# una-dinosauria/Rayuela.jl

Hardware: AMD Instinct MI355X
Metric: ADC queries/sec (linscan_pq, exact top-1000) (higher is better)
Workload: dtype f32; 1 GPU; SIFT1M-shape PQ m=8 h=256 encode + ADC linscan; n_base_total=1000000, n_base_per_gpu=1000000, nq=10000, k=1000, d=128, m=8, h=256, generator=splitmix64 (rayuela.jl_amd/synth.py; seeds base 1234, codebooks 99, rotation 7), parallelism=single GPU

## Files before the change

### include/rayuela_hip.h

```cpp
#ifndef RAYUELA_HIP_H_
#define RAYUELA_HIP_H_

#include <stddef.h>
#include <stdint.h>

#ifdef __cplusplus
extern "C" {
#endif

#define RQ_OK 0
#define RQ_EINVAL (-1)
#define RQ_EUNSUPPORTED (-2)
#define RQ_ENODEVICE (-3)

#define RQ_MAX_H16 32767
#define RQ_MAX_K 65536

const char *rq_version(void);
const char *rq_last_error(void);
int rq_device_count(void);
int rq_set_device(int device);

void linscan_aqd_query(float *dists, unsigned int *res, unsigned char *codes, float *centers,
                       float *queries, int N, unsigned int NQ, int B, int K, int dim1codes,
// ... 119 lines not shown
int rq_encode_opq_bytes_i16(int16_t *codes1, const uint8_t *X, const float *R, const float *C, int64_t n,
                            int d, int m, int h);
typedef struct rq_dataset rq_dataset;
rq_dataset *rq_dataset_upload(const float *X, int64_t n, int d);
rq_dataset *rq_dataset_upload_bytes(const uint8_t *X, int64_t n, int d);
int rq_dataset_encode(rq_dataset *ds, uint8_t *codes, int16_t *codes1, const float *R, const float *C, int m, int h);
void rq_dataset_free(rq_dataset *ds);
int rq_rotate_T(float *RX, const float *R, const float *X, int d, int64_t n);

int rq_dev_encode_pq(uint8_t *codes, const float *X, const float *C, int64_t n, int d, int m,
                     int h, void *stream);
int rq_dev_rotate_T(float *RX, const float *R, const float *X, int d, int64_t n, void *stream);
const char *rq_last_encode_kernel(void);
int rq_last_encode_stats(uint64_t *out2);
const char *rq_last_scan_kernel(void);
int rq_dev_encode_pq_filter_w(uint8_t *codes, float *W, const float *X, const float *C, int64_t n, int d, int m,
                              int h, void *stream);
int rq_dev_encode_opq(uint8_t *codes, const float *X, const float *R, const float *C, int64_t n,
                      int d, int m, int h, void *stream);
int rq_dev_encode_pq_bytes(uint8_t *codes, const uint8_t *X, const float *C, int64_t n, int d, int m,
                           int h, void *stream);
int rq_dev_encode_opq_bytes(uint8_t *codes, const uint8_t *X, const float *R, const float *C, int64_t n,
                            int d, int m, int h, void *stream);
int rq_dev_rotate_T_bytes(float *RX, const float *R, const uint8_t *X, int d, int64_t n, void *stream);
int rq_dev_encode_pq_wide(int16_t *codes, const float *X, const float *C, int64_t n, int d, int m, int h, void *stream);
int rq_dev_encode_opq_wide(int16_t *codes, const float *X, const float *R, const float *C, int64_t n, int d, int m, int h,
                           void *stream);
int rq_dev_encode_rvq_wide(int16_t *codes, float *Xr, const float *codebooks, int64_t n, int d, int m, int h,
                           uint32_t *counts, void *stream);
int rq_dev_adc_lut(float *lut, const float *centers, const float *queries, int64_t nq, int m,
// ... 67 lines not shown
```

### rayuela.jl_amd/_lib.py

```python
import ctypes as C

import numpy as np
import os

_HERE = os.path.dirname(os.path.abspath(__file__))


class RayuelaHipError(RuntimeError):
    pass


def lib_path():
    return os.environ.get("RAYUELA_HIP_LIB", os.path.join(_HERE, "librayuela_hip.so"))


_vp, _i32, _i64, _u32, _u64 = C.c_void_p, C.c_int, C.c_int64, C.c_uint32, C.c_uint64

SIGNATURES = {
    "rq_version": (C.c_char_p, []),
    "rq_last_scan_kernel": (C.c_char_p, []),
    "rq_last_error": (C.c_char_p, []),
    "rq_device_count": (_i32, []),
    "rq_set_device": (_i32, [_i32]),
    "linscan_aqd_query": (None, [_vp, _vp, _vp, _vp, _vp, _i32, C.c_uint, _i32, _i32, _i32, _i32, _i32]),
    "linscan_aqd_query_extra_byte": (None, [_vp, _vp, _vp, _vp, _vp, _vp, _i32, _i32, _i32, _i32, _i32, _i32]),
    "linscan_aqd_cq_query_extra_byte": (None, [_vp, _vp, _vp, _vp, _vp, _i32, _i32, _i32, _i32, _i32, _i32]),
    "rq_linscan_lsq": (_i32, [_vp, _vp, _vp, _vp, _vp, _vp, _vp, _i64, _i64, _i32, _i32, _i32, _i32, _i32]),
    "rq_linscan_cq": (_i32, [_vp, _vp, _vp, _vp, _vp, _i64, _i64, _i32, _i32, _i32, _i32, _i32]),
    "rq_lsq_prepare": (_vp, [_vp, _vp, _vp, _i64, _i32, _i32, _i32]),
    "rq_lsq_search": (_i32, [_vp, _vp, _vp, _vp, _vp, _i64, _i32, _i32]),
    "rq_lsq_release": (None, [_vp]),
    "rq_lsq_prepare_cbnorms": (_vp, [_vp, _vp, _vp, _i32, _i64, _i32, _i32, _i32]),
    "rq_aq_norms": (_i32, [_vp, _vp, _vp, _i64, _i32, _i32, _i32]),
    "rq_dev_aq_norms": (_i32, [_vp, _vp, _vp, _i64, _i32, _i32, _i32, _vp]),
    "rq_quantize_norms": (_i32, [_vp, _vp, _vp, _vp, _vp, _i64, _i32, _i32, _i32, _i32]),
# ... 217 lines not shown
```

### rayuela.jl_amd/csrc/rq_api.hip

```cpp
#include <stdarg.h>
#include <stdlib.h>
#include <string.h>

#include <chrono>
#include <mutex>
#include <string>
#include <thread>

#include <vector>
#include "rq_internal.h"

namespace rq {

static thread_local char g_err[512] = "";
static thread_local unsigned g_err_seq = 0;
static thread_local double g_t_total = 0, g_t_h2d = 0, g_t_kernel = 0, g_t_d2h = 0;

int fail(int code, const char *fmt, ...) {
  va_list ap;
  va_start(ap, fmt);
  vsnprintf(g_err, sizeof(g_err), fmt, ap);
  va_end(ap);
  ++g_err_seq;
  return code;
// ... 350 lines not shown
  RQ_TRY(order_cache_of(stream, &h, &og, &sg));
  if (sg != 0) {
    void *state = nullptr;
    RQ_TRY(workspace(WS_ORDER_STATE, order_cache_state_bytes(), &state, stream));
    RQ_HIP(hipMemsetAsync(state, 0, 8 * sizeof(uint32_t), stream));
  }
  h->key_id = 0;
  ++h->uncached;
  order_set_call_queries(nq);
  const int orc = order_base(ocodes, operm, ord, codes, n, mp, stream);
  order_set_call_queries(0);
  return orc;
}

static int order_kept(bool *kept, const uint8_t **ocodes, const uint32_t **operm, const uint8_t *codes, int64_t n, int m, int mp,
                      int64_t nq, size_t snap_off, hipStream_t stream) {
  *kept = true;
  OrderTiling ot;
  scan_order_tiling(mp, &ot);
  const int bits = order_cached_key_bits(n, mp, ot);
  if (bits <= 0) return RQ_OK;
  void *ord = nullptr, *state = nullptr, *tmp = nullptr;
  int rc = workspace(WS_ORDER, snap_off + (size_t)n * mp, &ord, stream);
  if (is_oom(rc)) { forgive_oom(); *kept = false; return RQ_OK; }
  RQ_TRY(rc);
  RQ_TRY(workspace(WS_ORDER_STATE, order_cache_state_bytes(), &state, stream));
  RQ_TRY(workspace(WS_ORDER_TMP, order_scratch_bytes(n, bits), &tmp, stream));
  OrderCacheHost *h = nullptr;
  uint64_t og = 0, sg = 0;
  RQ_TRY(order_cache_of(stream, &h, &og, &sg));
  if (h->state_gen != sg) {
    RQ_HIP(hipMemsetAsync(state, 0, order_cache_state_bytes(), stream));
    h->state_gen = sg; h->order_gen = og; h->key_id = 0;
  } else if (h->order_gen != og) {
    RQ_HIP(hipMemsetAsync(state, 0, 8 * sizeof(uint32_t), stream));
    h->order_gen = og; h->key_id = 0;
  }
  ++h->consulted;
  uint8_t *dst = (uint8_t *)ord;
  uint32_t *pm = reinterpret_cast<uint32_t *>(dst + (order_base_bytes(n, mp) - (size_t)n * 4));
  RQ_TRY(order_rows_cached(dst, pm, dst + snap_off, codes, n, m, mp, tmp, ot, nq, (uint32_t *)state, h, stream));
  *ocodes = dst;
  *operm = pm;
  return RQ_OK;
}

int order_cache_stats(unsigned long long *out8) {
  if (!out8) return fail(RQ_EINVAL, "rq_order_cache_stats: null output");
  int dev = 0;
  RQ_HIP(hipGetDevice(&dev));
  DeviceLock launch_lock;
  RQ_HIP(hipDeviceSynchronize());
  std::lock_guard<std::mutex> lk(g_mu);
  DevCtx &c = g_dev[dev];
  for (int i = 0; i < 8; ++i) out8[i] = 0;
  for (int i = 0; i < MAX_STREAM_WS; ++i) {
// ... 16 lines not shown
  const bool padded = base && (base->padded || base->perm);
  if (nq <= 0) return RQ_OK;
  if (n < 1 || n >= (1LL << 31)) return fail(RQ_EINVAL, "n=%lld must be in [1, 2^31)", (long long)n);
  if (lut_mode < LUT_PQ || lut_mode > LUT_CQ) return fail(RQ_EINVAL, "lut_mode=%d", lut_mode);
  if (m < 1 || d < 1 || (lut_mode == LUT_PQ && (d < m || d % m != 0)))
    return fail(RQ_EINVAL, "scan needs d %% m == 0 (src/Linscan.jl:23 Cint(d/m)); got d=%d m=%d", d, m);
  if (k < 1) return fail(RQ_EUNSUPPORTED, "k=%d outside [1, n]", k);
  if (k > n) return fail(RQ_EINVAL, "k=%d > n=%lld (undefined in the reference, deps/src/linscan_aqd.cpp:91)", k, (long long)n);
  if ((uint64_t)id_offset + (uint64_t)n > 0xFFFFFFFFull) return fail(RQ_EINVAL, "row ids overflow uint32");
  if (id_base != 0 && id_base != 1) return fail(RQ_EINVAL, "id_base must be 0 or 1");
  if (!keys && (!dists || !ids)) return fail(RQ_EINVAL, "need dists+ids or keys");
  if (((uintptr_t)codes & 15) != 0) return fail(RQ_EINVAL, "codes pointer must be 16-byte aligned");
  DeviceInfo di;
  RQ_TRY(device_info(&di));
  DeviceLock launch_lock;
  const int mp = scan_padded_m(m);
  if (mp < 0) return fail(RQ_EUNSUPPORTED, "the ADC scan kernels cover 1 <= m <= 64 sub-quantizers; got m=%d", m);
  if (mp != m && !padded) {
    void *padded = nullptr;
    RQ_TRY(workspace(WS_PAD, (size_t)n * mp, &padded, stream));
    RQ_TRY(pad_codes_launch((uint8_t *)padded, codes, n, m, mp, stream));
    codes = (const uint8_t *)padded;
  }
  if (k > RQ_MAX_K)
    return bulk_scan(dists, ids, keys, codes, centers, queries, n, nq, m, d, k, id_offset, id_base, stream, lut_mode, row_bias,
                     perm, di.num_cu);
  const size_t order_cap = (size_t)std::max(0, tuning("ORDER_MAX_SCRATCH_MB", 2048)) * 1048576ull;
  if (!perm && !row_bias && order_pays(n, nq, k) && order_base_bytes(n, mp) + (size_t)n * 4 <= order_cap) {
    const uint8_t *ocodes = codes;
    const uint32_t *operm = nullptr;
    const size_t snap_off = (order_base_bytes(n, mp) + 255) & ~(size_t)255, snap_bytes = (size_t)n * mp;
    bool kept = false;
    int orc = RQ_OK;
    if (snap_off + snap_bytes + (size_t)n * 4 <= order_cap) orc = order_kept(&kept, &ocodes, &operm, codes, n, m, mp, nq, snap_off, stream);
    if (orc == RQ_OK && !kept) orc = order_in_call(&ocodes, &operm, codes, n, mp, nq, stream);
    if (orc == RQ_OK) {
      codes = ocodes;
      perm = operm;
    } else if (is_oom(orc)) {
      forgive_oom();
    } else {
      return orc;
    }
  }
  ScanPlan pl;
  RQ_TRY(scan_plan(pl, n, nq, m, d, k, di.num_cu, tuning("SCAN_SLICES", 0)));
  void *cand = nullptr, *counter = nullptr;
  RQ_TRY(workspace(WS_CAND, pl.cand_bytes, &cand, stream));
  RQ_TRY(workspace(WS_COUNTER, WS_COUNTER_BYTES, &counter, stream));
  const int64_t q_tail = std::min<int64_t>(nq, (int64_t)pl.whole * pl.qg);
  const bool sliced = pl.nslices > 1 && q_tail < nq;
  const bool both = keys && (dists || ids);
  void *part = nullptr;
  if (sliced) RQ_TRY(workspace(WS_KEYS, (size_t)(nq - q_tail) * pl.nslices * k * sizeof(uint64_t), &part, stream));
  void *normb = norm_prepared;
  if (lut_mode == LUT_LSQ && row_bias && !normb)
    RQ_TRY(workspace(WS_NORMB, lsq_norm_bytes(n), &normb, stream));
  RQ_TRY(scan_launch(pl, both ? nullptr : dists, both ? nullptr : ids, keys, (uint64_t *)part, codes, centers, queries,
                     n, nq, m, d, k, id_offset, id_base, (uint32_t *)counter, (uint64_t *)cand, stream, lut_mode,
                     row_bias, (uint8_t *)normb, perm, norm_prepared != nullptr));
  if (sliced) {
    const size_t off = (size_t)q_tail * k;
    RQ_TRY(merge_launch(both || !dists ? nullptr : dists + off, both || !ids ? nullptr : ids + off,
                        keys ? keys + off : nullptr, (const uint64_t *)part, nq - q_tail, (int)pl.nslices, k, id_base,
                        stream));
  }
  if (both) return merge_launch(dists, ids, nullptr, keys, nq, 1, k, id_base, stream);
  return RQ_OK;
}

template <class ScanFn>
static int scan_and_fetch(float *dists, uint32_t *ids, float *dd, uint32_t *di, int64_t nq, int k, ScanFn scan) {
  const int64_t hc = std::max(256, tuning("HOST_CHUNK", 4096));
  const int64_t chunk = (nq >= 2 * hc && tuning("HOST_OVERLAP", 1)) ? hc : nq;
  const size_t row = (size_t)k * 4;
// ... 326 lines not shown
  g_t_kernel = std::max(0.0, g_t_total - h2d - tail);
  return RQ_OK;
}

}

using namespace rq;

extern "C" {

#ifndef RQ_BUILD_ID
#define RQ_BUILD_ID "unknown"
#endif
const char *rq_version(void) { return "rayuela-hip 0.1 (gfx950) build " RQ_BUILD_ID; }
const char *rq_last_scan_kernel(void) { return last_scan_kernel_name(); }
const char *rq_last_error(void) { return g_err; }

int rq_device_count(void) {
  int n = 0;
  if (hipGetDeviceCount(&n) != hipSuccess) { (void)hipGetLastError(); return 0; }
  return n;
}

int rq_set_device(int device) {
  RQ_HIP(hipSetDevice(device));
  return RQ_OK;
}

int rq_set_tuning(const char *key, int value) {
  if (!key || !*key) return fail(RQ_EINVAL, "rq_set_tuning: empty key");
// ... 774 lines not shown
```

### rayuela.jl_amd/csrc/rq_internal.h

```cpp
#pragma once
#include <hip/hip_runtime.h>
#include <stdint.h>
#include <stdio.h>

#include <math.h>

#include <algorithm>

#include "../../include/rayuela_hip.h"

namespace rq {

int fail(int code, const char *fmt, ...) __attribute__((format(printf, 2, 3)));
int fail_hip(hipError_t e, const char *what, const char *file, int line);
inline bool is_oom(int rc) { return rc == (int)hipErrorOutOfMemory; }
void forgive_oom();

#define RQ_HIP(expr)                                                       \
  do {                                                                     \
    hipError_t _e = (expr);                                                \
    if (_e != hipSuccess) return ::rq::fail_hip(_e, #expr, __FILE__, __LINE__); \
  } while (0)

#define RQ_TRY(expr)            \
// ... 44 lines not shown
void set_timing(double total_ms, double h2d_ms, double kernel_ms, double d2h_ms);

struct ScanPlan {
  int qg, blk;
  uint32_t ngroups, nslices, rows_per_slice, whole;
  uint32_t cap, trigger, p2, scratch_keys, grid, sample;
  size_t cand_bytes, gtab_off, bkt_off;
  bool lds_ok, bigk, spread;
  bool xcd;
};
int scan_plan(ScanPlan &pl, int64_t n, int64_t nq, int m, int d, int K, int num_cu, int force_slices);
int scan_launch(const ScanPlan &pl, float *dists, uint32_t *ids, uint64_t *keys, uint64_t *part, const uint8_t *codes,
                const float *centers, const float *queries, int64_t n, int64_t nq, int m, int d, int K,
                uint32_t id_offset, int id_base, uint32_t *work_counter, uint64_t *cand,
                hipStream_t stream, int lut_mode = 0, const float *row_bias = nullptr, uint8_t *norm_buf = nullptr,
                const uint32_t *perm = nullptr, bool norm_ready = false);
const char *last_scan_kernel_name();
void set_last_scan_kernel(const char *name);
size_t lsq_norm_bytes(int64_t n);
int lsq_norm_prepare(uint8_t *norm_buf, const uint8_t *codes, const float *centers, const float *row_bias, int64_t n,
                     int mp, int m_real, int d, hipStream_t stream);
enum { LUT_PQ = 0, LUT_LSQ = 1, LUT_CQ = 2 };
struct ScanBase {
  const uint32_t *perm = nullptr;
  uint8_t *norm_prepared = nullptr;
  bool padded = false;
};
int dev_linscan(float *dists, uint32_t *ids, uint64_t *keys, const uint8_t *codes, const float *centers,
                const float *queries, int64_t n, int64_t nq, int m, int d, int k, uint32_t id_offset,
                int id_base, hipStream_t stream, int lut_mode = LUT_PQ, const float *row_bias = nullptr,
                const ScanBase *base = nullptr);
bool order_pays(int64_t n, int64_t nq, int k);
// ... 10 lines not shown
int order_sample_stride();
uint32_t order_sample_rows(int64_t n, int blk, uint32_t *sgroups);
int gather_f32_launch(float *dst, const float *src, const uint32_t *perm, int64_t n, hipStream_t stream);
int order_rows_launch(uint8_t *dst, uint32_t *perm, const uint8_t *src, int64_t n, int mp, void *scratch,
                      const OrderTiling &t, hipStream_t stream);
struct OrderCacheHost {
  unsigned char key[768];
  uint32_t key_id = 0;
  uint32_t epoch = 0;
  uint64_t order_gen = 0, state_gen = 0;
  unsigned long long consulted = 0, uncached = 0;
};
size_t order_cache_state_bytes();
int order_cached_key_bits(int64_t n, int mp, const OrderTiling &t);
int order_rows_cached(uint8_t *dst, uint32_t *perm, uint8_t *snap, const uint8_t *src, int64_t n, int m, int mp, void *scratch,
                      const OrderTiling &t, int64_t nq, uint32_t *state, OrderCacheHost *h, hipStream_t stream);
int order_cache_stats(unsigned long long *out8);
int interleave_keys_launch(uint64_t *dst, const uint64_t *src, int64_t nq, int P, int k, size_t pstride, hipStream_t stream);
int scan_padded_m(int m);
int pad_codes_launch(uint8_t *dst, const uint8_t *src, int64_t n, int m, int mp, hipStream_t stream);
constexpr size_t BULK_SCRATCH_BYTES = (size_t)2 << 30;
constexpr size_t BULK_HOST_RESULT_BYTES = (size_t)256 << 20;
int bulk_scan(float *dists, uint32_t *ids, uint64_t *keys, const uint8_t *codes, const float *centers, const float *queries,
              int64_t n, int64_t nq, int m, int d, int k, uint32_t id_offset, int id_base, hipStream_t stream, int lut_mode,
              const float *row_bias, const uint32_t *perm, int num_cu);
int bulk_merge(float *dists, uint32_t *ids, uint64_t *keys_out, const uint64_t *keys_in, int64_t nq, int P, int K,
               int id_base, hipStream_t stream);
void bulk_plan(int64_t n, int64_t nq, int m, int k, int num_cu, int64_t *qg, int64_t *groups, int64_t *grid, int64_t *batch);
int merge_launch(float *dists, uint32_t *ids, uint64_t *keys_out, const uint64_t *keys_in, int64_t nq,
                 int P, int K, int id_base, hipStream_t stream);
int lut_launch(float *lut, const float *centers, const float *queries, int64_t nq, int m, int sub,
// ... 96 lines not shown
```

### rayuela.jl_amd/csrc/rq_order.hip

```cpp
#include "rq_internal.h"

#include <cmath>
#include <cstring>
#include <mutex>

namespace rq {

struct OrderParams {
  const uint8_t *src;
  uint8_t *dst;
  uint32_t *perm;
  uint32_t *rank;
  uint32_t *hist;
  uint32_t n;
  int mp;
  int ncoord;
  int nb[8];
  uint32_t nbins;
  uint32_t tile;
  uint32_t rpt;
  uint32_t group;
  uint32_t gran;
  uint32_t ngran;
  uint32_t weyl;
// ... 76 lines not shown
  if (lead) {
    g.state[OC_VERDICT] = v; g.state[OC_VEPOCH] = g.epoch;
    if (v == OCV_REBUILD) { g.state[OC_BUILT] = 0; g.state[OC_CNT + (g.balanced ? 2 : 1)] += 1; }
    else if (v == OCV_HIT) g.state[OC_CNT] += 1;
  }
  return v == OCV_REBUILD;
}
__device__ __forceinline__ bool order_gate_open(const OrderGate &g) {
  return !g.state || (g.state[OC_VEPOCH] == g.epoch && g.state[OC_VERDICT] == (g.role == 2 ? OCV_UPGRADE : OCV_REBUILD));
}
__device__ __forceinline__ bool order_gate_last(const OrderGate &g) {
  if (!order_gate_open(g)) return false;
  if (g.state && blockIdx.x == 0 && threadIdx.x == 0) { g.state[OC_BALANCED] = g.balanced; g.state[OC_BUILT] = g.key; }
  return true;
}
__device__ __forceinline__ void order_snapshot(const OrderGate &g, const uint8_t *src, size_t bytes) {
  if (!g.state || !g.snap || g.role != 1) return;
  const size_t nv = bytes / 16, nth = (size_t)gridDim.x * blockDim.x, t0 = (size_t)blockIdx.x * blockDim.x + threadIdx.x;
  for (size_t i = t0; i < nv; i += nth) reinterpret_cast<uint4 *>(g.snap)[i] = reinterpret_cast<const uint4 *>(src)[i];
  if (t0 == 0) for (size_t b = nv * 16; b < bytes; ++b) g.snap[b] = src[b];
}

__global__ __launch_bounds__(256) void order_check_kernel(const uint8_t *codes, const uint8_t *snap, size_t bytes, uint32_t *state,
                                                          uint32_t key, uint32_t epoch, uint32_t *zero, uint32_t nzero) {
  const size_t nth = (size_t)gridDim.x * blockDim.x, t0 = (size_t)blockIdx.x * blockDim.x + threadIdx.x;
  for (size_t i = t0; i < nzero; i += nth) zero[i] = 0u;
  if (state[OC_BUILT] != key) return;
  const size_t nv = bytes / 16;
  bool bad = false;
  for (size_t i = t0; i < nv; i += nth) {
    const uint4 a = reinterpret_cast<const uint4 *>(codes)[i], b = reinterpret_cast<const uint4 *>(snap)[i];
    bad |= ((a.x ^ b.x) | (a.y ^ b.y) | (a.z ^ b.z) | (a.w ^ b.w)) != 0u;
  }
  if (t0 == 0) for (size_t b = nv * 16; b < bytes; ++b) bad |= codes[b] != snap[b];
  if (bad) state[OC_MISS] = epoch;
}

__global__ __launch_bounds__(256) void order_zero_kernel(OrderParams p, uint32_t count, OrderGate g) {
  if (!order_gate_first(g)) return;
  order_snapshot(g, p.src, (size_t)p.n * p.mp);
  for (uint32_t i = blockIdx.x * blockDim.x + threadIdx.x; i < count; i += gridDim.x * blockDim.x) p.hist[i] = 0u;
// ... 92 lines not shown
      const uint32_t y = __shfl_up(x, off);
      if ((tid & 63u) >= (uint32_t)off) x += y;
    }
    if ((tid & 63u) == 63u) wsum[tid >> 6] = x;
  }
  __syncthreads();
  if (tid < ORDER_COARSE) {
    uint32_t base = 0;
    for (uint32_t w = 0; w < (tid >> 6); ++w) base += wsum[w];
    starts[tid] = base + x - v;
    if (tid == ORDER_COARSE - 1) starts[ORDER_COARSE] = base + x;
  }
  __syncthreads();
}

__global__ __launch_bounds__(ORDER_SMALL_THREADS) void order_coarse_count_kernel(OrderParams p, OrderSmall q, OrderGate g) {
  __shared__ uint32_t h[ORDER_COARSE];
  const uint32_t tid = threadIdx.x;
  if (!order_gate_first(g)) return;
  order_snapshot(g, p.src, (size_t)p.n * p.mp);
  if (tid < ORDER_COARSE) h[tid] = 0;
  __syncthreads();
  const uint32_t r0 = blockIdx.x * q.rows_per_wg, r1 = min(p.n, r0 + q.rows_per_wg);
  for (uint32_t i = r0 + tid; i < r1; i += ORDER_SMALL_THREADS)
    if (!order_in_prefix(p, i)) atomicAdd(&h[order_key_of(p, i) >> q.fine_bits], 1u);
  __syncthreads();
  if (tid < ORDER_COARSE && h[tid]) atomicAdd(&q.ctot[tid], h[tid]);
}

__global__ __launch_bounds__(ORDER_SMALL_THREADS) void order_coarse_scatter_kernel(OrderParams p, OrderSmall q, OrderGate g) {
  __shared__ uint32_t h[ORDER_COARSE], base[ORDER_COARSE], starts[ORDER_COARSE + 1];
  const uint32_t tid = threadIdx.x;
  if (!order_gate_open(g)) return;
  if (tid < ORDER_COARSE) h[tid] = 0;
  coarse_starts(starts, q.ctot);
  const uint32_t r0 = blockIdx.x * q.rows_per_wg, r1 = min(p.n, r0 + q.rows_per_wg);
  constexpr int PER = 4;
  uint32_t c[PER], lr[PER];
#pragma unroll
  for (int u = 0; u < PER; ++u) {
    const uint32_t i = r0 + u * ORDER_SMALL_THREADS + tid;
    c[u] = 0xffffffffu;
    if (i < r1) {
      if (order_in_prefix(p, i)) order_copy_row(p, i, order_sample_pos(p, i / p.stride));
      else { c[u] = order_key_of(p, i) >> q.fine_bits; lr[u] = atomicAdd(&h[c[u]], 1u); }
    }
  }
  __syncthreads();
  if (tid < ORDER_COARSE && h[tid]) base[tid] = starts[tid] + atomicAdd(&q.ctot[ORDER_COARSE + tid], h[tid]);
  __syncthreads();
#pragma unroll
  for (int u = 0; u < PER; ++u) {
    const uint32_t i = r0 + u * ORDER_SMALL_THREADS + tid;
    if (c[u] != 0xffffffffu) q.idx[base[c[u]] + lr[u]] = i;
  }
}

__global__ __launch_bounds__(ORDER_SMALL_THREADS) void order_fine_kernel(OrderParams p, OrderSmall q, OrderGate g) {
  __shared__ uint32_t f[ORDER_FINE_MAX], starts[ORDER_COARSE + 1], wsum[16];
  const uint32_t tid = threadIdx.x, nfine = 1u << q.fine_bits, fmask = nfine - 1u;
  if (!order_gate_last(g)) return;
  for (uint32_t i = tid; i < nfine; i += ORDER_SMALL_THREADS) f[i] = 0;
  coarse_starts(starts, q.ctot);
  const uint32_t b0 = starts[blockIdx.x], b1 = starts[blockIdx.x + 1];
  for (uint32_t i = b0 + tid; i < b1; i += ORDER_SMALL_THREADS) atomicAdd(&f[order_key_of(p, q.idx[i]) & fmask], 1u);
  __syncthreads();
  {
    const uint32_t v = tid < nfine ? f[tid] : 0u;
    uint32_t x = v;
#pragma unroll
// ... 90 lines not shown
#pragma unroll
        for (int i = 0; i < TPL; ++i)
          mine_st[i * 128 + (val[i] & 31u)] = (uint16_t)(((x[i] & 255u) + (fresh[i] ? 1u : 0u)) | (val[i] << 8));
        next += 1u;
      }
      myrank = lane == j ? newrank : myrank;
      __builtin_amdgcn_wave_barrier();
    }
    if (have) order_copy_row(p, row, order_deal(p, myrank));
    row = row_n;
#pragma unroll
    for (uint32_t i = 0; i < NW; ++i) w[i] = w_n[i];
  }
}

__global__ __launch_bounds__(ORDER_SMALL_THREADS) void order_fine_greedy_kernel(OrderParams p, OrderSmall q, OrderGate g) {
  __shared__ uint32_t f[ORDER_FINE_MAX], fst[ORDER_FINE_MAX + 1], starts[ORDER_COARSE + 1], wsum[16];
  extern __shared__ __attribute__((aligned(16))) uint32_t dyn[];
  const uint32_t tid = threadIdx.x, nfine = 1u << q.fine_bits, fmask = nfine - 1u;
  if (!order_gate_last(g)) return;
  for (uint32_t i = tid; i < nfine; i += ORDER_SMALL_THREADS) f[i] = 0;
  coarse_starts(starts, q.ctot);
  const uint32_t b0 = starts[blockIdx.x], b1 = starts[blockIdx.x + 1];
  const bool fits = b1 - b0 <= p.glist;
  for (uint32_t i = b0 + tid; i < b1; i += ORDER_SMALL_THREADS) atomicAdd(&f[order_key_of(p, q.idx[i]) & fmask], 1u);
  __syncthreads();
  {
    const uint32_t v = tid < nfine ? f[tid] : 0u;
    uint32_t x = v;
#pragma unroll
    for (int off = 1; off < 64; off <<= 1) {
      const uint32_t y = __shfl_up(x, off);
      if ((tid & 63u) >= (uint32_t)off) x += y;
    }
    if ((tid & 63u) == 63u) wsum[tid >> 6] = x;
    __syncthreads();
    uint32_t wb = 0;
    for (uint32_t w = 0; w < (tid >> 6); ++w) wb += wsum[w];
    if (tid < nfine) { f[tid] = b0 + wb + x - v; fst[tid] = b0 + wb + x - v; }
// ... 15 lines not shown
  }
  __syncthreads();
  const uint32_t wave = tid >> 6;
  if (wave >= p.gwaves) return;
  uint16_t *st = reinterpret_cast<uint16_t *>(reinterpret_cast<uint8_t *>(dyn + p.glist) + (size_t)wave * GREEDY_GROUPS * (uint32_t)p.gfree * 64u);
  const uint32_t window = GREEDY_GROUPS * p.group;
  for (uint32_t fb = wave; fb < nfine; fb += p.gwaves) {
    const uint32_t s0 = fst[fb], s1 = fst[fb + 1];
    for (uint32_t c0 = s0; c0 < s1;) {
      const uint32_t c1 = min(s1, c0 / p.group * p.group + window);
      if (p.mp == 8) greedy_chunk<8, 1>(p, list, b0, c0, c1, st);
      else greedy_chunk<16, 3>(p, list, b0, c0, c1, st);
      c0 = c1;
    }
  }
}

static uint32_t gcd_u32(uint32_t a, uint32_t b) { while (b) { const uint32_t t = a % b; a = b; b = t; } return a; }

int order_sample_stride() { return tuning("ORDER_SAMPLE_STRIDE", 16); }

uint32_t order_sample_rows(int64_t n, int blk, uint32_t *sgroups) {
  const int stride = order_sample_stride();
  uint32_t g = 0;
  if (stride >= 2 && blk > 0) g = (uint32_t)(n / ((int64_t)stride * blk));
  if (sgroups) *sgroups = g;
  return g * (uint32_t)blk;
}

static thread_local int64_t g_order_call_nq = 0;
// ... 114 lines not shown
    const OrderSmall &q = s.q;
    const uint32_t nwg = (uint32_t)((n + q.rows_per_wg - 1) / q.rows_per_wg);
    if (zero_counters) RQ_HIP(hipMemsetAsync(q.ctot, 0, 2 * ORDER_COARSE * 4, stream));
    hipLaunchKernelGGL(order_coarse_count_kernel, dim3(nwg), dim3(ORDER_SMALL_THREADS), 0, stream, p, q, g);
    RQ_HIP(hipGetLastError());
    hipLaunchKernelGGL(order_coarse_scatter_kernel, dim3(nwg), dim3(ORDER_SMALL_THREADS), 0, stream, p, q, g);
    RQ_HIP(hipGetLastError());
    if (s.greedy) {
      RQ_HIP(hipFuncSetAttribute(reinterpret_cast<const void *>(order_fine_greedy_kernel),
                                 hipFuncAttributeMaxDynamicSharedMemorySize, (int)s.lds));
      hipLaunchKernelGGL(order_fine_greedy_kernel, dim3(ORDER_COARSE), dim3(ORDER_SMALL_THREADS), s.lds, stream, p, q, g);
    } else {
      hipLaunchKernelGGL(order_fine_kernel, dim3(ORDER_COARSE), dim3(ORDER_SMALL_THREADS), 0, stream, p, q, g);
    }
    RQ_HIP(hipGetLastError());
    return RQ_OK;
  }
  const uint32_t ntiles = (p.nbins + ORDER_SCAN_TILE - 1) / ORDER_SCAN_TILE;
  const uint32_t grid = (uint32_t)std::min<int64_t>((n + 255) / 256, 256 * 16);
  if (g.state) {
    hipLaunchKernelGGL(order_zero_kernel, dim3(grid), dim3(256), 0, stream, p, p.nbins + ntiles, g);
    RQ_HIP(hipGetLastError());
  } else if (zero_counters) {
    RQ_HIP(hipMemsetAsync(p.hist, 0, (size_t)(p.nbins + ntiles) * 4, stream));
  }
  hipLaunchKernelGGL(order_rank_kernel, dim3(grid), dim3(256), 0, stream, p, g);
  RQ_HIP(hipGetLastError());
  hipLaunchKernelGGL(order_scan_tiles_kernel, dim3(ntiles), dim3(1024), 0, stream, p.hist, p.nbins, g);
  RQ_HIP(hipGetLastError());
  hipLaunchKernelGGL(order_scan_top_kernel, dim3(1), dim3(1024), 0, stream, p.hist + p.nbins, ntiles, g);
  RQ_HIP(hipGetLastError());
  hipLaunchKernelGGL(order_scatter_kernel, dim3(grid), dim3(256), 0, stream, p, g);
  RQ_HIP(hipGetLastError());
  return RQ_OK;
}

int order_rows_launch(uint8_t *dst, uint32_t *perm, const uint8_t *src, int64_t n, int mp, void *scratch,
                      const OrderTiling &t, hipStream_t stream) {
  OrderSet s;
  RQ_TRY(order_plan_set(s, n, mp, t));
  order_bind(s, dst, perm, src, scratch);
  OrderGate g;
  memset(&g, 0, sizeof(g));
  return order_run_set(s, g, true, stream);
}

struct OrderCacheKey {
  int64_t n;
// ... 1 lines not shown
  OrderSet plain, bal;
};
static_assert(sizeof(OrderCacheKey) <= sizeof(OrderCacheHost::key), "OrderCacheHost::key too small");

size_t order_cache_state_bytes() { return OC_WORDS * sizeof(uint32_t); }

int order_cached_key_bits(int64_t n, int mp, const OrderTiling &t) {
  int nb[8];
  order_set_call_queries(-1);
  const int bits = order_key_bits(n, mp, t, nb);
  order_set_call_queries(0);
  return bits;
}

int order_rows_cached(uint8_t *dst, uint32_t *perm, uint8_t *snap, const uint8_t *src, int64_t n, int m, int mp, void *scratch,
                      const OrderTiling &t, int64_t nq, uint32_t *state, OrderCacheHost *h, hipStream_t stream) {
  static uint32_t next_id = 0;
  static std::mutex id_mu;
  OrderCacheKey key;
  memset(&key, 0, sizeof(key));
  key.n = n; key.m = m; key.mp = mp;
  order_set_call_queries(-1);
  int rc = order_plan_set(key.plain, n, mp, t);
  order_set_call_queries(0);
  if (rc == RQ_OK) rc = order_plan_set(key.bal, n, mp, t);
  if (rc != RQ_OK) return rc;
  key.has_b = key.bal.greedy ? 1 : 0;
  if (!key.has_b) memset(&key.bal, 0, sizeof(key.bal));
  if (h->key_id == 0 || memcmp(h->key, &key, sizeof(key)) != 0) {
    std::lock_guard<std::mutex> lk(id_mu);
    if (++next_id == 0) ++next_id;
    h->key_id = next_id;
    memcpy(h->key, &key, sizeof(key));
  }
  if (++h->epoch == 0) ++h->epoch;
  const bool first_bal = key.has_b && !(nq > 0 && nq < tuning("ORDER_GREEDY_MIN_NQ", 16384));
  OrderSet first = first_bal ? key.bal : key.plain;
  order_bind(first, dst, perm, src, scratch);
  OrderGate g;
  memset(&g, 0, sizeof(g));
  g.state = state; g.snap = snap; g.key = h->key_id; g.epoch = h->epoch;
  g.role = 1; g.can_upgrade = key.has_b; g.balanced = first_bal;
  const size_t bytes = (size_t)n * mp;
  const uint32_t cgrid = (uint32_t)std::max<size_t>(1, std::min<size_t>((bytes / 16 + 511) / 512, 2048));
  const bool zero2 = first.two_level || g.can_upgrade;
  hipLaunchKernelGGL(order_check_kernel, dim3(cgrid), dim3(256), 0, stream, src, (const uint8_t *)snap, bytes, state, g.key, g.epoch,
                     reinterpret_cast<uint32_t *>(scratch) + n, zero2 ? 2u * ORDER_COARSE : 0u);
  RQ_HIP(hipGetLastError());
  RQ_TRY(order_run_set(first, g, false, stream));
  if (g.can_upgrade) {
    OrderSet up = key.bal;
    order_bind(up, dst, perm, src, scratch);
    g.role = 2; g.can_upgrade = 0; g.balanced = 1;
    RQ_TRY(order_run_set(up, g, false, stream));
  }
  return RQ_OK;
}

__global__ void gather_f32_kernel(float *__restrict__ dst, const float *__restrict__ src, const uint32_t *__restrict__ perm, uint32_t n) {
  for (uint32_t i = blockIdx.x * blockDim.x + threadIdx.x; i < n; i += gridDim.x * blockDim.x) dst[i] = src[perm[i]];
}

int gather_f32_launch(float *dst, const float *src, const uint32_t *perm, int64_t n, hipStream_t stream) {
  if (n <= 0) return RQ_OK;
  hipLaunchKernelGGL(gather_f32_kernel, dim3((uint32_t)std::min<int64_t>((n + 255) / 256, 4096)), dim3(256), 0, stream, dst, src, perm, (uint32_t)n);
  RQ_HIP(hipGetLastError());
  return RQ_OK;
}

}
```

### rayuela.jl_amd/csrc/rq_scan.hip

```cpp
#include "rq_internal.h"
#include "rq_topk.h"

#include "rq_scan_tables.h"
#include "rq_scan_filter.h"
#include "rq_scan_select.h"


namespace rq {

#define RQ_STAT_T() ((p.stats && threadIdx.x == 0) ? (unsigned long long)clock64() : 0ull)
#define RQ_STAT_ADD(slot, t0) do { if (p.stats && threadIdx.x == 0) atomicAdd(&p.stats[slot], (unsigned long long)clock64() - (t0)); } while (0)
#define RQ_STAT_INC(slot) do { if (p.stats && threadIdx.x == 0) atomicAdd(&p.stats[slot], 1ull); } while (0)

struct BucketFinishArgs {
  uint32_t cap, scratch_keys, nq, K, id_base;
  int bfin;
  float *dists;
  uint32_t *ids;
  unsigned long long *stats;
};
template <int M>
__device__ __noinline__ bool bucket_finish_item(ScanCtrl<ScanCfg<M>::QG> *ctrl_g, uint64_t *cand_wg, BucketFinishArgs p,
                                                uint64_t *scratch_g, int g, int gi, uint32_t q0, uint64_t *keys_base,
                                                uint32_t key_stride, uint32_t vseq_in, uint32_t *vseq_out) {
// ... 724 lines not shown
  const int lim = (int)((nbytes - i) < 8 ? (nbytes - i) : 8);
  for (int b = 0; b < lim; ++b) {
    uint64_t z = ((e0 + i + b) ^ seed) + 0x9E3779B97F4A7C15ull;
    z = (z ^ (z >> 30)) * 0xBF58476D1CE4E5B9ull;
    z = (z ^ (z >> 27)) * 0x94D049BB133111EBull;
    z = z ^ (z >> 31);
    out |= (z >> 56) << (8 * b);
  }
  if (lim == 8) *reinterpret_cast<uint64_t *>(codes + i) = out;
  else for (int b = 0; b < lim; ++b) codes[i + b] = (uint8_t)(out >> (8 * b));
}

static thread_local char g_last_scan_kernel[64] = "";
const char *last_scan_kernel_name() { return g_last_scan_kernel; }
void set_last_scan_kernel(const char *name) { snprintf(g_last_scan_kernel, sizeof(g_last_scan_kernel), "%s", name); }

template <int M>
static int launch_scan(ScanParams &p, const ScanPlan &plan, hipStream_t stream) {
  using Cfg = ScanCfg<M>;
  p.samp_end = 0; p.samp_stride = 16;
  if (p.perm) {
    uint32_t groups = 0;
    (void)order_sample_rows((int64_t)p.n, Cfg::BLK, &groups);
    p.samp_stride = (uint32_t)std::max(2, order_sample_stride());
    p.samp_end = groups * p.samp_stride * (uint32_t)Cfg::BLK;
  }
  constexpr int CTRL_BYTES = (sizeof(ScanCtrl<Cfg::QG>) + 15) & ~15;
  size_t lds = CTRL_BYTES + (size_t)std::max<size_t>(Cfg::LUT_LDS_BYTES + (size_t)Cfg::QG * p.d * 4 + Cfg::AUX_BYTES,
                                                     (size_t)p.scratch_keys * 8);
  if (p.bigk) lds = std::max<size_t>(lds, CTRL_BYTES + SS_LDS_BYTES);
// ... 191 lines not shown
  RQ_HIP(hipMemsetAsync(cn, 0, 16 * 256 * 4, stream));
  const uint32_t grid = (uint32_t)std::min<int64_t>(2048, (n + 255) / 256);
  hipLaunchKernelGGL(cnorm_kernel, dim3((m_real * 256 + 255) / 256), dim3(256), 0, stream, centers, m_real * 256, d, cn);
  hipLaunchKernelGGL(norm_residual_kernel, dim3(grid), dim3(256), 0, stream, row_bias, codes, (uint32_t)n, mp, m_real, cn, rho);
  hipLaunchKernelGGL(norm_minmax_kernel, dim3(grid), dim3(256), 0, stream, (const float *)rho, (uint32_t)n, info);
  hipLaunchKernelGGL(norm_info_kernel, dim3(1), dim3(1), 0, stream, info);
  hipLaunchKernelGGL(norm_quant_kernel, dim3(grid), dim3(256), 0, stream, (const float *)rho, (uint32_t)n, info, norm_buf);
  RQ_HIP(hipGetLastError());
  return RQ_OK;
}

int scan_launch(const ScanPlan &pl, float *dists, uint32_t *ids, uint64_t *keys, uint64_t *part, const uint8_t *codes,
                const float *centers, const float *queries, int64_t n, int64_t nq, int m, int d, int K,
                uint32_t id_offset, int id_base, uint32_t *work_counter, uint64_t *cand,
                hipStream_t stream, int lut_mode, const float *row_bias, uint8_t *norm_buf, const uint32_t *perm,
                bool norm_ready) {
  ScanParams p;
  p.perm = perm;
  p.samp_end = 0;
  p.codes = codes; p.centers = centers; p.queries = queries;
  p.n = (uint32_t)n; p.nq = (uint32_t)nq; p.sub = d / m; p.d = d; p.K = K;
  p.m_real = m;
  m = scan_padded_m(m);
  p.lut_mode = lut_mode; p.row_bias = row_bias;
  p.id_offset = id_offset; p.id_base = id_base;
  p.nslices = pl.nslices; p.rows_per_slice = pl.rows_per_slice; p.ngroups = pl.ngroups; p.whole = pl.whole;
  p.xcd_mode = pl.xcd ? 1u : 0u;
  {
    const uint32_t per_xcd = std::max(1u, pl.grid / 8u);
    const int rd = tuning("SCAN_XCD_ROUND", 0);
    p.xcd_round = rd > 0 ? (uint32_t)rd : pl.ngroups * ((per_xcd + pl.ngroups - 1u) / pl.ngroups);
// ... 22 lines not shown
  p.norm_bytes = nullptr; p.norm_info = nullptr; p.cnorm = nullptr;
  if (lut_mode == LUT_LSQ && row_bias && norm_buf && (m == 8 || m == 16) && tuning("SCAN_FILTER", 1) &&
      tuning("SCAN_FILTER_LSQ", 1)) {
    if (!norm_ready) RQ_TRY(lsq_norm_prepare(norm_buf, codes, centers, row_bias, n, m, p.m_real, d, stream));
    const size_t nb_bytes = ((size_t)n + 63) & ~(size_t)63;
    uint32_t *info = reinterpret_cast<uint32_t *>(norm_buf + nb_bytes);
    float *cn = reinterpret_cast<float *>(info + 8);
    p.norm_bytes = norm_buf;
    p.norm_info = reinterpret_cast<const float *>(info) + 4;
    p.cnorm = cn;
    p.filter = 1;
  }
  p.stats = tuning("SCAN_STATS", 0) ? reinterpret_cast<unsigned long long *>(work_counter + 16) : nullptr;
  p.dists = dists; p.ids = ids; p.keys = keys; p.part = part;
#if RQ_SCAN_PACE_BUILD
  if (p.pace) RQ_HIP(hipMemsetAsync(work_counter + 64, 0, WS_COUNTER_BYTES - 256, stream));
#endif
  RQ_HIP(hipMemsetAsync(work_counter, 0, p.stats ? 256 : 16 * sizeof(uint32_t), stream));
  switch (m) {
    case 2: return launch_scan<2>(p, pl, stream);
    case 4: return launch_scan<4>(p, pl, stream);
    case 8: return launch_scan<8>(p, pl, stream);
    case 16: return launch_scan<16>(p, pl, stream);
    case 32: return launch_scan<32>(p, pl, stream);
    case 64: return launch_scan<64>(p, pl, stream);
  }
  return fail(RQ_EUNSUPPORTED, "m=%d", m);
}

int merge_launch(float *dists, uint32_t *ids, uint64_t *keys_out, const uint64_t *keys_in, int64_t nq,
                 int P, int K, int id_base, hipStream_t stream) {
  if (P > 1 && K > RQ_MAX_K) return bulk_merge(dists, ids, keys_out, keys_in, nq, P, K, id_base, stream);
  MergeParams p;
// ... 79 lines not shown
```

Baseline: 5.503 million queries/s.

## Fuse order-cache first and upgrade passes and fold counter zeroing into check

The cached row-ordering path now runs the first and balanced-upgrade orderings as one set of three gated kernels that pick their parameter set from a device-side verdict, instead of launching both sets back to back. The scan work counter is zeroed inside the order check kernel, so the separate hipMemsetAsync before the scan is skipped when that happened. The aim is fewer kernel launches and memsets in front of the scan for each query batch, at the cost of more complex gate state handling. A launch counter API is added so the front launches can be inspected.

```diff
diff --git a/include/rayuela_hip.h b/include/rayuela_hip.h
--- a/include/rayuela_hip.h
+++ b/include/rayuela_hip.h
@@ -157,6 +157,7 @@
 const char *rq_last_encode_kernel(void);
 int rq_last_encode_stats(uint64_t *out2);
 const char *rq_last_scan_kernel(void);
+int rq_scan_front_launches(void);
 int rq_dev_encode_pq_filter_w(uint8_t *codes, float *W, const float *X, const float *C, int64_t n, int d, int m,
                               int h, void *stream);
 int rq_dev_encode_opq(uint8_t *codes, const float *X, const float *R, const float *C, int64_t n,
diff --git a/rayuela.jl_amd/_lib.py b/rayuela.jl_amd/_lib.py
--- a/rayuela.jl_amd/_lib.py
+++ b/rayuela.jl_amd/_lib.py
@@ -19,6 +19,7 @@
 SIGNATURES = {
     "rq_version": (C.c_char_p, []),
     "rq_last_scan_kernel": (C.c_char_p, []),
+    "rq_scan_front_launches": (_i32, []),
     "rq_last_error": (C.c_char_p, []),
     "rq_device_count": (_i32, []),
     "rq_set_device": (_i32, [_i32]),
diff --git a/rayuela.jl_amd/csrc/rq_api.hip b/rayuela.jl_amd/csrc/rq_api.hip
--- a/rayuela.jl_amd/csrc/rq_api.hip
+++ b/rayuela.jl_amd/csrc/rq_api.hip
@@ -388,8 +388,9 @@
 }
 
 static int order_kept(bool *kept, const uint8_t **ocodes, const uint32_t **operm, const uint8_t *codes, int64_t n, int m, int mp,
-                      int64_t nq, size_t snap_off, hipStream_t stream) {
+                      int64_t nq, size_t snap_off, uint32_t *counter, bool *zeroed, hipStream_t stream) {
   *kept = true;
+  *zeroed = false;
   OrderTiling ot;
   scan_order_tiling(mp, &ot);
   const int bits = order_cached_key_bits(n, mp, ot);
@@ -413,7 +414,8 @@
   ++h->consulted;
   uint8_t *dst = (uint8_t *)ord;
   uint32_t *pm = reinterpret_cast<uint32_t *>(dst + (order_base_bytes(n, mp) - (size_t)n * 4));
-  RQ_TRY(order_rows_cached(dst, pm, dst + snap_off, codes, n, m, mp, tmp, ot, nq, (uint32_t *)state, h, stream));
+  RQ_TRY(order_rows_cached(dst, pm, dst + snap_off, codes, n, m, mp, tmp, ot, nq, (uint32_t *)state, h, counter, 16u, stream));
+  *zeroed = counter != nullptr;
   *ocodes = dst;
   *operm = pm;
   return RQ_OK;
@@ -460,6 +462,7 @@
   DeviceInfo di;
   RQ_TRY(device_info(&di));
   DeviceLock launch_lock;
+  FrontLaunchScope front_scope(!base);
   const int mp = scan_padded_m(m);
   if (mp < 0) return fail(RQ_EUNSUPPORTED, "the ADC scan kernels cover 1 <= m <= 64 sub-quantizers; got m=%d", m);
   if (mp != m && !padded) {
@@ -467,18 +470,25 @@
     RQ_TRY(workspace(WS_PAD, (size_t)n * mp, &padded, stream));
     RQ_TRY(pad_codes_launch((uint8_t *)padded, codes, n, m, mp, stream));
     codes = (const uint8_t *)padded;
+    front_launches_add(1);
   }
   if (k > RQ_MAX_K)
     return bulk_scan(dists, ids, keys, codes, centers, queries, n, nq, m, d, k, id_offset, id_base, stream, lut_mode, row_bias,
                      perm, di.num_cu);
   const size_t order_cap = (size_t)std::max(0, tuning("ORDER_MAX_SCRATCH_MB", 2048)) * 1048576ull;
+  void *cand = nullptr, *counter = nullptr;
+  bool counter_zeroed = false;
   if (!perm && !row_bias && order_pays(n, nq, k) && order_base_bytes(n, mp) + (size_t)n * 4 <= order_cap) {
     const uint8_t *ocodes = codes;
     const uint32_t *operm = nullptr;
     const size_t snap_off = (order_base_bytes(n, mp) + 255) & ~(size_t)255, snap_bytes = (size_t)n * mp;
     bool kept = false;
     int orc = RQ_OK;
-    if (snap_off + snap_bytes + (size_t)n * 4 <= order_cap) orc = order_kept(&kept, &ocodes, &operm, codes, n, m, mp, nq, snap_off, stream);
+    if (snap_off + snap_bytes + (size_t)n * 4 <= order_cap) {
+      RQ_TRY(workspace(WS_COUNTER, WS_COUNTER_BYTES, &counter, stream));
+      orc = order_kept(&kept, &ocodes, &operm, codes, n, m, mp, nq, snap_off, (uint32_t *)counter, &counter_zeroed, stream);
+      if (orc != RQ_OK || !kept) counter_zeroed = false;
+    }
     if (orc == RQ_OK && !kept) orc = order_in_call(&ocodes, &operm, codes, n, mp, nq, stream);
     if (orc == RQ_OK) {
       codes = ocodes;
@@ -491,7 +501,6 @@
   }
   ScanPlan pl;
   RQ_TRY(scan_plan(pl, n, nq, m, d, k, di.num_cu, tuning("SCAN_SLICES", 0)));
-  void *cand = nullptr, *counter = nullptr;
   RQ_TRY(workspace(WS_CAND, pl.cand_bytes, &cand, stream));
   RQ_TRY(workspace(WS_COUNTER, WS_COUNTER_BYTES, &counter, stream));
   const int64_t q_tail = std::min<int64_t>(nq, (int64_t)pl.whole * pl.qg);
@@ -504,7 +513,7 @@
     RQ_TRY(workspace(WS_NORMB, lsq_norm_bytes(n), &normb, stream));
   RQ_TRY(scan_launch(pl, both ? nullptr : dists, both ? nullptr : ids, keys, (uint64_t *)part, codes, centers, queries,
                      n, nq, m, d, k, id_offset, id_base, (uint32_t *)counter, (uint64_t *)cand, stream, lut_mode,
-                     row_bias, (uint8_t *)normb, perm, norm_prepared != nullptr));
+                     row_bias, (uint8_t *)normb, perm, norm_prepared != nullptr, counter_zeroed));
   if (sliced) {
     const size_t off = (size_t)q_tail * k;
     RQ_TRY(merge_launch(both || !dists ? nullptr : dists + off, both || !ids ? nullptr : ids + off,
@@ -861,6 +870,7 @@
 #endif
 const char *rq_version(void) { return "rayuela-hip 0.1 (gfx950) build " RQ_BUILD_ID; }
 const char *rq_last_scan_kernel(void) { return last_scan_kernel_name(); }
+int rq_scan_front_launches(void) { return front_launches(); }
 const char *rq_last_error(void) { return g_err; }
 
 int rq_device_count(void) {
diff --git a/rayuela.jl_amd/csrc/rq_internal.h b/rayuela.jl_amd/csrc/rq_internal.h
--- a/rayuela.jl_amd/csrc/rq_internal.h
+++ b/rayuela.jl_amd/csrc/rq_internal.h
@@ -82,8 +82,18 @@
                 const float *centers, const float *queries, int64_t n, int64_t nq, int m, int d, int K,
                 uint32_t id_offset, int id_base, uint32_t *work_counter, uint64_t *cand,
                 hipStream_t stream, int lut_mode = 0, const float *row_bias = nullptr, uint8_t *norm_buf = nullptr,
-                const uint32_t *perm = nullptr, bool norm_ready = false);
+                const uint32_t *perm = nullptr, bool norm_ready = false, bool counter_zeroed = false);
 const char *last_scan_kernel_name();
+void front_launches_begin(bool raw);
+void front_launches_end();
+void front_launches_add(int n);
+int front_launches();
+struct FrontLaunchScope {
+  explicit FrontLaunchScope(bool raw) { front_launches_begin(raw); }
+  ~FrontLaunchScope() { front_launches_end(); }
+  FrontLaunchScope(const FrontLaunchScope &) = delete;
+  FrontLaunchScope &operator=(const FrontLaunchScope &) = delete;
+};
 void set_last_scan_kernel(const char *name);
 size_t lsq_norm_bytes(int64_t n);
 int lsq_norm_prepare(uint8_t *norm_buf, const uint8_t *codes, const float *centers, const float *row_bias, int64_t n,
@@ -124,7 +134,8 @@
 size_t order_cache_state_bytes();
 int order_cached_key_bits(int64_t n, int mp, const OrderTiling &t);
 int order_rows_cached(uint8_t *dst, uint32_t *perm, uint8_t *snap, const uint8_t *src, int64_t n, int m, int mp, void *scratch,
-                      const OrderTiling &t, int64_t nq, uint32_t *state, OrderCacheHost *h, hipStream_t stream);
+                      const OrderTiling &t, int64_t nq, uint32_t *state, OrderCacheHost *h, uint32_t *zero2p, uint32_t nzero2,
+                      hipStream_t stream);
 int order_cache_stats(unsigned long long *out8);
 int interleave_keys_launch(uint64_t *dst, const uint64_t *src, int64_t nq, int P, int k, size_t pstride, hipStream_t stream);
 int scan_padded_m(int m);
diff --git a/rayuela.jl_amd/csrc/rq_order.hip b/rayuela.jl_amd/csrc/rq_order.hip
--- a/rayuela.jl_amd/csrc/rq_order.hip
+++ b/rayuela.jl_amd/csrc/rq_order.hip
@@ -114,17 +114,44 @@
   if (g.state && blockIdx.x == 0 && threadIdx.x == 0) { g.state[OC_BALANCED] = g.balanced; g.state[OC_BUILT] = g.key; }
   return true;
 }
+__device__ __forceinline__ uint32_t order_gate2_first(const OrderGate &g) {
+  const bool hit = g.state[OC_BUILT] == g.key && g.state[OC_MISS] != g.epoch;
+  const uint32_t v = !hit ? OCV_REBUILD : !g.state[OC_BALANCED] ? OCV_UPGRADE : OCV_HIT;
+  if (blockIdx.x == 0 && threadIdx.x == 0) {
+    g.state[OC_VERDICT] = v; g.state[OC_VEPOCH] = g.epoch;
+    if (v == OCV_REBUILD) { g.state[OC_BUILT] = 0; g.state[OC_CNT + (g.balanced ? 2 : 1)] += 1; }
+    else if (v == OCV_HIT) g.state[OC_CNT] += 1;
+  }
+  return v == OCV_HIT ? 0u : v;
+}
+__device__ __forceinline__ uint32_t order_gate2_open(const OrderGate &g) {
+  if (g.state[OC_VEPOCH] != g.epoch) return 0u;
+  const uint32_t v = g.state[OC_VERDICT];
+  return (v == OCV_REBUILD || v == OCV_UPGRADE) ? v : 0u;
+}
+__device__ __forceinline__ uint32_t order_gate2_second(const OrderGate &g) {
+  const uint32_t v = order_gate2_open(g);
+  if (v == OCV_UPGRADE && blockIdx.x == 0 && threadIdx.x == 0) { g.state[OC_BUILT] = 0; g.state[OC_CNT + 2] += 1; g.state[OC_CNT + 3] += 1; }
+  return v;
+}
+__device__ __forceinline__ uint32_t order_gate2_last(const OrderGate &g) {
+  const uint32_t v = order_gate2_open(g);
+  if (v && blockIdx.x == 0 && threadIdx.x == 0) { g.state[OC_BALANCED] = v == OCV_UPGRADE ? 1u : g.balanced; g.state[OC_BUILT] = g.key; }
+  return v;
+}
 __device__ __forceinline__ void order_snapshot(const OrderGate &g, const uint8_t *src, size_t bytes) {
-  if (!g.state || !g.snap || g.role != 1) return;
+  if (!g.state || !g.snap || g.role == 2) return;
   const size_t nv = bytes / 16, nth = (size_t)gridDim.x * blockDim.x, t0 = (size_t)blockIdx.x * blockDim.x + threadIdx.x;
   for (size_t i = t0; i < nv; i += nth) reinterpret_cast<uint4 *>(g.snap)[i] = reinterpret_cast<const uint4 *>(src)[i];
   if (t0 == 0) for (size_t b = nv * 16; b < bytes; ++b) g.snap[b] = src[b];
 }
 
 __global__ __launch_bounds__(256) void order_check_kernel(const uint8_t *codes, const uint8_t *snap, size_t bytes, uint32_t *state,
-                                                          uint32_t key, uint32_t epoch, uint32_t *zero, uint32_t nzero) {
+                                                          uint32_t key, uint32_t epoch, uint32_t *zero, uint32_t nzero,
+                                                          uint32_t *zero2, uint32_t nzero2) {
   const size_t nth = (size_t)gridDim.x * blockDim.x, t0 = (size_t)blockIdx.x * blockDim.x + threadIdx.x;
   for (size_t i = t0; i < nzero; i += nth) zero[i] = 0u;
+  for (size_t i = t0; i < nzero2; i += nth) zero2[i] = 0u;
   if (state[OC_BUILT] != key) return;
   const size_t nv = bytes / 16;
   bool bad = false;
@@ -247,11 +274,9 @@
   __syncthreads();
 }
 
-__global__ __launch_bounds__(ORDER_SMALL_THREADS) void order_coarse_count_kernel(OrderParams p, OrderSmall q, OrderGate g) {
+__device__ __forceinline__ void order_coarse_count_body(const OrderParams &p, const OrderSmall &q) {
   __shared__ uint32_t h[ORDER_COARSE];
   const uint32_t tid = threadIdx.x;
-  if (!order_gate_first(g)) return;
-  order_snapshot(g, p.src, (size_t)p.n * p.mp);
   if (tid < ORDER_COARSE) h[tid] = 0;
   __syncthreads();
   const uint32_t r0 = blockIdx.x * q.rows_per_wg, r1 = min(p.n, r0 + q.rows_per_wg);
@@ -261,10 +286,15 @@
   if (tid < ORDER_COARSE && h[tid]) atomicAdd(&q.ctot[tid], h[tid]);
 }
 
-__global__ __launch_bounds__(ORDER_SMALL_THREADS) void order_coarse_scatter_kernel(OrderParams p, OrderSmall q, OrderGate g) {
+__global__ __launch_bounds__(ORDER_SMALL_THREADS) void order_coarse_count_kernel(OrderParams p, OrderSmall q, OrderGate g) {
+  if (!order_gate_first(g)) return;
+  order_snapshot(g, p.src, (size_t)p.n * p.mp);
+  order_coarse_count_body(p, q);
+}
+
+__device__ __forceinline__ void order_coarse_scatter_body(const OrderParams &p, const OrderSmall &q) {
   __shared__ uint32_t h[ORDER_COARSE], base[ORDER_COARSE], starts[ORDER_COARSE + 1];
   const uint32_t tid = threadIdx.x;
-  if (!order_gate_open(g)) return;
   if (tid < ORDER_COARSE) h[tid] = 0;
   coarse_starts(starts, q.ctot);
   const uint32_t r0 = blockIdx.x * q.rows_per_wg, r1 = min(p.n, r0 + q.rows_per_wg);
@@ -287,6 +317,11 @@
     const uint32_t i = r0 + u * ORDER_SMALL_THREADS + tid;
     if (c[u] != 0xffffffffu) q.idx[base[c[u]] + lr[u]] = i;
   }
+}
+
+__global__ __launch_bounds__(ORDER_SMALL_THREADS) void order_coarse_scatter_kernel(OrderParams p, OrderSmall q, OrderGate g) {
+  if (!order_gate_open(g)) return;
+  order_coarse_scatter_body(p, q);
 }
 
 __global__ __launch_bounds__(ORDER_SMALL_THREADS) void order_fine_kernel(OrderParams p, OrderSmall q, OrderGate g) {
@@ -407,15 +442,13 @@
   }
 }
 
-__global__ __launch_bounds__(ORDER_SMALL_THREADS) void order_fine_greedy_kernel(OrderParams p, OrderSmall q, OrderGate g) {
+__device__ __forceinline__ void order_fine_greedy_body(const OrderParams &p, const OrderSmall &q, uint32_t *dyn) {
   __shared__ uint32_t f[ORDER_FINE_MAX], fst[ORDER_FINE_MAX + 1], starts[ORDER_COARSE + 1], wsum[16];
-  extern __shared__ __attribute__((aligned(16))) uint32_t dyn[];
   const uint32_t tid = threadIdx.x, nfine = 1u << q.fine_bits, fmask = nfine - 1u;
-  if (!order_gate_last(g)) return;
   for (uint32_t i = tid; i < nfine; i += ORDER_SMALL_THREADS) f[i] = 0;
   coarse_starts(starts, q.ctot);
   const uint32_t b0 = starts[blockIdx.x], b1 = starts[blockIdx.x + 1];
-  const bool fits = b1 - b0 <= p.glist;
+  const bool fits = p.gfree != 0 && b1 - b0 <= p.glist;
   for (uint32_t i = b0 + tid; i < b1; i += ORDER_SMALL_THREADS) atomicAdd(&f[order_key_of(p, q.idx[i]) & fmask], 1u);
   __syncthreads();
   {
@@ -461,6 +494,40 @@
       c0 = c1;
     }
   }
+}
+
+__global__ __launch_bounds__(ORDER_SMALL_THREADS) void order_fine_greedy_kernel(OrderParams p, OrderSmall q, OrderGate g) {
+  extern __shared__ __attribute__((aligned(16))) uint32_t dyn[];
+  if (!order_gate_last(g)) return;
+  order_fine_greedy_body(p, q, dyn);
+}
+
+struct OrderPair {
+  OrderParams p[2];
+  OrderSmall q[2];
+};
+
+__global__ __launch_bounds__(ORDER_SMALL_THREADS) void order2_count_kernel(OrderPair pr, OrderGate g) {
+  const uint32_t v = order_gate2_first(g);
+  if (!v) return;
+  const uint32_t s = v == OCV_UPGRADE ? 1u : 0u;
+  if (!s) order_snapshot(g, pr.p[0].src, (size_t)pr.p[0].n * pr.p[0].mp);
+  order_coarse_count_body(pr.p[s], pr.q[s]);
+}
+
+__global__ __launch_bounds__(ORDER_SMALL_THREADS) void order2_scatter_kernel(OrderPair pr, OrderGate g) {
+  const uint32_t v = order_gate2_second(g);
+  if (!v) return;
+  const uint32_t s = v == OCV_UPGRADE ? 1u : 0u;
+  order_coarse_scatter_body(pr.p[s], pr.q[s]);
+}
+
+__global__ __launch_bounds__(ORDER_SMALL_THREADS) void order2_fine_kernel(OrderPair pr, OrderGate g) {
+  extern __shared__ __attribute__((aligned(16))) uint32_t dyn[];
+  const uint32_t v = order_gate2_last(g);
+  if (!v) return;
+  const uint32_t s = v == OCV_UPGRADE ? 1u : 0u;
+  order_fine_greedy_body(pr.p[s], pr.q[s], dyn);
 }
 
 static uint32_t gcd_u32(uint32_t a, uint32_t b) { while (b) { const uint32_t t = a % b; a = b; b = t; } return a; }
@@ -605,6 +672,7 @@
       hipLaunchKernelGGL(order_fine_kernel, dim3(ORDER_COARSE), dim3(ORDER_SMALL_THREADS), 0, stream, p, q, g);
     }
     RQ_HIP(hipGetLastError());
+    front_launches_add(zero_counters ? 4 : 3);
     return RQ_OK;
   }
   const uint32_t ntiles = (p.nbins + ORDER_SCAN_TILE - 1) / ORDER_SCAN_TILE;
@@ -623,6 +691,26 @@
   RQ_HIP(hipGetLastError());
   hipLaunchKernelGGL(order_scatter_kernel, dim3(grid), dim3(256), 0, stream, p, g);
   RQ_HIP(hipGetLastError());
+  front_launches_add((g.state || zero_counters) ? 5 : 4);
+  return RQ_OK;
+}
+
+static int order_run_pair(const OrderSet &first, const OrderSet &up, const OrderGate &g, hipStream_t stream) {
+  OrderPair pr;
+  pr.p[0] = first.p; pr.q[0] = first.q;
+  pr.p[1] = up.p; pr.q[1] = up.q;
+  const uint32_t nwg = (uint32_t)(((int64_t)first.p.n + first.q.rows_per_wg - 1) / first.q.rows_per_wg);
+  const uint32_t lds = std::max(first.lds, up.lds);
+  hipLaunchKernelGGL(order2_count_kernel, dim3(nwg), dim3(ORDER_SMALL_THREADS), 0, stream, pr, g);
+  RQ_HIP(hipGetLastError());
+  front_launches_add(1);
+  hipLaunchKernelGGL(order2_scatter_kernel, dim3(nwg), dim3(ORDER_SMALL_THREADS), 0, stream, pr, g);
+  RQ_HIP(hipGetLastError());
+  front_launches_add(1);
+  RQ_HIP(hipFuncSetAttribute(reinterpret_cast<const void *>(order2_fine_kernel), hipFuncAttributeMaxDynamicSharedMemorySize, (int)lds));
+  hipLaunchKernelGGL(order2_fine_kernel, dim3(ORDER_COARSE), dim3(ORDER_SMALL_THREADS), lds, stream, pr, g);
+  RQ_HIP(hipGetLastError());
+  front_launches_add(1);
   return RQ_OK;
 }
 
@@ -654,7 +742,8 @@
 }
 
 int order_rows_cached(uint8_t *dst, uint32_t *perm, uint8_t *snap, const uint8_t *src, int64_t n, int m, int mp, void *scratch,
-                      const OrderTiling &t, int64_t nq, uint32_t *state, OrderCacheHost *h, hipStream_t stream) {
+                      const OrderTiling &t, int64_t nq, uint32_t *state, OrderCacheHost *h, uint32_t *zero2p, uint32_t nzero2,
+                      hipStream_t stream) {
   static uint32_t next_id = 0;
   static std::mutex id_mu;
   OrderCacheKey key;
@@ -685,16 +774,19 @@
   const uint32_t cgrid = (uint32_t)std::max<size_t>(1, std::min<size_t>((bytes / 16 + 511) / 512, 2048));
   const bool zero2 = first.two_level || g.can_upgrade;
   hipLaunchKernelGGL(order_check_kernel, dim3(cgrid), dim3(256), 0, stream, src, (const uint8_t *)snap, bytes, state, g.key, g.epoch,
-                     reinterpret_cast<uint32_t *>(scratch) + n, zero2 ? 2u * ORDER_COARSE : 0u);
+                     reinterpret_cast<uint32_t *>(scratch) + n, zero2 ? 2u * ORDER_COARSE : 0u, zero2p, zero2p ? nzero2 : 0u);
   RQ_HIP(hipGetLastError());
+  front_launches_add(1);
+  if (!g.can_upgrade) return order_run_set(first, g, false, stream);
+  OrderSet up = key.bal;
+  order_bind(up, dst, perm, src, scratch);
+  if (first.two_level && up.two_level) {
+    g.role = 3;
+    return order_run_pair(first, up, g, stream);
+  }
   RQ_TRY(order_run_set(first, g, false, stream));
-  if (g.can_upgrade) {
-    OrderSet up = key.bal;
-    order_bind(up, dst, perm, src, scratch);
-    g.role = 2; g.can_upgrade = 0; g.balanced = 1;
-    RQ_TRY(order_run_set(up, g, false, stream));
-  }
-  return RQ_OK;
+  g.role = 2; g.can_upgrade = 0; g.balanced = 1;
+  return order_run_set(up, g, false, stream);
 }
 
 __global__ void gather_f32_kernel(float *__restrict__ dst, const float *__restrict__ src, const uint32_t *__restrict__ perm, uint32_t n) {
diff --git a/rayuela.jl_amd/csrc/rq_scan.hip b/rayuela.jl_amd/csrc/rq_scan.hip
--- a/rayuela.jl_amd/csrc/rq_scan.hip
+++ b/rayuela.jl_amd/csrc/rq_scan.hip
@@ -762,6 +762,12 @@
 static thread_local char g_last_scan_kernel[64] = "";
 const char *last_scan_kernel_name() { return g_last_scan_kernel; }
 void set_last_scan_kernel(const char *name) { snprintf(g_last_scan_kernel, sizeof(g_last_scan_kernel), "%s", name); }
+static thread_local int g_front_launches = 0;
+static thread_local bool g_front_counting = false;
+void front_launches_begin(bool raw) { g_front_counting = raw; if (raw) g_front_launches = 0; }
+void front_launches_end() { g_front_counting = false; }
+void front_launches_add(int n) { if (g_front_counting) g_front_launches += n; }
+int front_launches() { return g_front_launches; }
 
 template <int M>
 static int launch_scan(ScanParams &p, const ScanPlan &plan, hipStream_t stream) {
@@ -983,7 +989,7 @@
                 const float *centers, const float *queries, int64_t n, int64_t nq, int m, int d, int K,
                 uint32_t id_offset, int id_base, uint32_t *work_counter, uint64_t *cand,
                 hipStream_t stream, int lut_mode, const float *row_bias, uint8_t *norm_buf, const uint32_t *perm,
-                bool norm_ready) {
+                bool norm_ready, bool counter_zeroed) {
   ScanParams p;
   p.perm = perm;
   p.samp_end = 0;
@@ -1036,9 +1042,12 @@
   p.stats = tuning("SCAN_STATS", 0) ? reinterpret_cast<unsigned long long *>(work_counter + 16) : nullptr;
   p.dists = dists; p.ids = ids; p.keys = keys; p.part = part;
 #if RQ_SCAN_PACE_BUILD
-  if (p.pace) RQ_HIP(hipMemsetAsync(work_counter + 64, 0, WS_COUNTER_BYTES - 256, stream));
+  if (p.pace) { RQ_HIP(hipMemsetAsync(work_counter + 64, 0, WS_COUNTER_BYTES - 256, stream)); front_launches_add(1); counter_zeroed = false; }
 #endif
-  RQ_HIP(hipMemsetAsync(work_counter, 0, p.stats ? 256 : 16 * sizeof(uint32_t), stream));
+  if (!counter_zeroed || p.stats) {
+    RQ_HIP(hipMemsetAsync(work_counter, 0, p.stats ? 256 : 16 * sizeof(uint32_t), stream));
+    front_launches_add(1);
+  }
   switch (m) {
     case 2: return launch_scan<2>(p, pl, stream);
     case 4: return launch_scan<4>(p, pl, stream);
```

Measured after the change: 5.522 million queries/s, median of 6. No clear change (+0.3%).
